# revdotcom/paper_accurate_fast_cheap

Hardware: AMD Instinct MI355X
Metric: audio-sec/sec (1/RTF) GigaSpeech long-form encode (higher is better)
Workload: dtype f32+bf16-slot

## Files before the change

include/pafc_encoder_ops.h:

```cpp
#ifndef PAFC_ENCODER_OPS_H
#define PAFC_ENCODER_OPS_H

#include "pafc_wkv6.h"

#ifdef __cplusplus
extern "C" {
#endif

int pafc_dwconv1d_cl(int dtype, int B, int T_in, int C, int K, int left_pad, int T_out, const void *x,
                     const void *w, const void *bias, void *y, int glu, const int32_t *lens,
                     pafc_stream_t stream);

int pafc_dwconv1d_cl_ex(int dtype, int B, int T_in, int C, int K, int left_pad, int T_out, const void *x, long ldx,
                        const void *w, const void *bias, void *y, int act, const int32_t *lens, pafc_stream_t stream);

int pafc_dwconv1d_cl_ln_silu(int dtype, int B, int T_in, int C, int K, int left_pad, int T_out, const void *x, long ldx,
                             const void *w, const void *bias, const void *gamma, const void *beta, float eps, void *y,
                             const int32_t *lens, pafc_stream_t stream);

size_t pafc_dwconv1d_cl_wgrad_workspace_bytes(int B, int T_out, int C, int K);
int pafc_dwconv1d_cl_wgrad(int dtype, int B, int T_in, int C, int K, int left_pad, int T_out, const void *x, long ldx,
                           const void *dy, float *dw, float *dbias, void *workspace, size_t workspace_bytes,
                           pafc_stream_t stream);

// ... 143 lines not shown
size_t pafc_mamba2_scan_workspace_bytes(int B, int L, int H, int chunk_len);
int pafc_mamba2_scan(int B, int L, int H, const void *xbc, long ldx, const float *dt, const float *log_a, float *y,
                     int chunk_len, void *workspace, size_t workspace_bytes, pafc_stream_t stream);
int pafc_mamba2_scan_dir(int B, int L, int H, const void *xbc, long ldx, const float *dt, const float *log_a, float *y,
                         int reverse, int chunk_len, void *workspace, size_t workspace_bytes, pafc_stream_t stream);

int pafc_mamba2_scan_skip_bf16(int B, int L, int H, const void *xbc, long ldx, const float *dt, const float *log_a,
                               const float *D, void *y_bf16, int reverse, int chunk_len, void *workspace,
                               size_t workspace_bytes, pafc_stream_t stream);
int pafc_mamba2_gate_norm(int dtype, long rows, int d_inner, const void *y, const void *z, long ld_z,
                          const void *norm_weight, float eps, void *out, pafc_stream_t stream);

int pafc_mamba2_scan_state(int B, int L, int H, const void *xbc, long ldx, const float *dt, const float *log_a, const float *D,
                           float *y_f32, void *y_bf16, const float *s_in, float *s_out, int reverse, int chunk_len,
                           void *workspace, size_t workspace_bytes, pafc_stream_t stream);

int pafc_gemm_bf16(long M, int N, int K, int batch, const void *A, long lda, long strideA, const void *W, long ldw,
                   long strideW, const void *bias, long strideBias, const void *residual, long ldr, long strideR,
                   void *out, long ldo, long strideO, float alpha, int act, pafc_stream_t stream);
int pafc_gemm_bf16_glu_half(long M, int N, int K, int batch);
int pafc_conv3x3s2_nhwc_bf16_ph(int B, int T1, int F1, int Ci, int Co, const void *in, const void *w_tap_co_ci, const void *bias,
                                void *out, int relu, int tile_m, pafc_stream_t stream);
int pafc_gemm_bf16_ph(long M, int N, int K, int batch, const void *A, long lda, long strideA, const void *W, long ldw,
                      long strideW, const void *bias, long strideBias, const void *residual, long ldr, long strideR,
                      void *out, long ldo, long strideO, float alpha, int act, int tile_n, int tile_m, pafc_stream_t stream);
int pafc_gemm_ph_ex(long M, int N, int K, int batch, const void *A, long lda, long strideA, int a_split, const void *W, long ldw,
                    long strideW, const void *bias, long strideBias, const void *residual, int res_kind, long ldr, long strideR,
                    void *out, int out_kind, long ldo, long lo_off, long strideO, float alpha, int act, int tile_m,
                    pafc_stream_t stream);
int pafc_gemm_ph_ex2(long M, int N, int K, int batch, const void *A, long lda, long strideA, int a_split, int a_plane_block,
                     const void *W, long ldw, long strideW, const void *bias, long strideBias, const void *residual, int res_kind,
                     long ldr, long strideR, void *out, int out_kind, long ldo, long lo_off, long strideO, float alpha, int act,
                     int tile_m, pafc_stream_t stream);
int pafc_conv3x3s2_nhwc_split_ph(int B, int T1, int F1, int Ci, int Co, const void *in_planes, const void *w3_tap_co_3ci,
                                 const float *bias, void *out_planes, int relu, int tile_m, pafc_stream_t stream);

int pafc_residual_dropout(int backward, int dtype_x, int dtype_y, long n, const void *x, const void *y, void *out, float scale,
                          float p, unsigned long long seed, unsigned long long offset, pafc_stream_t stream);
int pafc_silu_dropout(int backward, int dtype, long n, const void *h, const void *dout, void *out, float p,
                      unsigned long long seed, unsigned long long offset, pafc_stream_t stream);

int pafc_multi_transpose_bf16(const void *table, int n, int total_tiles, pafc_stream_t stream);
int pafc_multi_cast_bf16(const void *table, int n, int total_chunks, pafc_stream_t stream);

#ifdef __cplusplus
}
#endif
#endif
```

paper_accurate_fast_cheap_amd/_lib.py:

```python
import ctypes
import os
from ctypes import c_float, c_int, c_long, c_size_t, c_ulonglong, c_void_p

import torch

_HERE = os.path.dirname(os.path.abspath(__file__))
SO_PATH = os.path.join(_HERE, "libpafc_hip.so")

PAFC_F32, PAFC_BF16 = 0, 1
_ERRORS = {
    -1: "null pointer", -2: "bad dims (B, T, C, H must be positive and C == H * 64)", -3: "head size must be 64",
    -4: "workspace too small", -5: "kernel launch failed", -6: "unsupported dtype", -7: "unsupported",
    -8: "r, k, v, w, y must be 16-byte aligned",
}


class PafcError(RuntimeError):
    pass


_lib = None


def lib():
# ... 58 lines not shown
    "pafc_conv3x3s2_c1_nhwc_f32split": (I, [I, I, I, I, P, P, P, P, P, I, P]),
    "pafc_conv3x3s2_c1_nhwc_f32split_ps": (I, [I, I, I, I, P, P, P, P, P, G, I, P]),
    "pafc_conv3x3s2_nhwc_f32split": (I, [I, I, I, I, I, P, P, P, P, P, P, I, P]),
    "pafc_gemm_tn_workspace_bytes": (Z, [G, I, I]),
    "pafc_gemm_tn_bf16": (I, [G, I, I, P, G, P, G, P, P, I, P, Z, P]),
    "pafc_gemm_tn_batched_workspace_bytes": (Z, [G, I, I, I]),
    "pafc_gemm_tn_bf16_batched": (I, [G, I, I, I, P, G, G, P, G, G, P, P, I, P, Z, P]),
    "pafc_gemm_bf16_f32out": (I, [G, I, I, P, G, I, P, G, P, P, G, P, I, G, G, F, I, P, Z, P]),
    "pafc_gemm_bf16_f32out_pb": (I, [G, I, I, P, G, I, I, P, G, P, P, G, P, I, G, G, F, I, P, Z, P]),
    "pafc_gemm_bf16_f32out_workspace_bytes": (Z, [G, I, I, I]),
    "pafc_ctc_loss_workspace_bytes": (Z, [I, I, I]),
    "pafc_ctc_loss_forward": (I, [I, I, I, I, P, G, P, P, I, P, I, I, P, P, Z, P]),
    "pafc_ctc_loss_backward": (I, [I, I, I, I, P, G, P, P, I, P, I, I, P, P, F, P, G, P, Z, P]),
    "pafc_rnnt_joint_loss_workspace_bytes": (Z, [I, I, I, G, G, P, I]),
    "pafc_rnnt_joint_loss_forward": (I, [I, I, I, I, I, P, G, G, P, G, G, P, P, P, P, P, I, I, G, P, P, Z, P]),
    "pafc_rnnt_joint_loss_backward": (I, [I, I, I, I, I, P, G, G, P, G, G, P, P, P, P, P, I, I, G, P, G, P, F, I, P, P, P, P,
        P, Z, P, Z, P]),
    "pafc_gemm_f32": (I, [G, I, I, I, P, G, G, P, G, G, P, G, P, G, G, P, G, G, F, I, P]),
    "pafc_mamba2_prep": (I, [I, I, I, I, P, P, G, P, P, P, P, P, P, P, P, P]),
    "pafc_mamba2_finish": (I, [I, I, I, I, P, P, P, P, G, P, G, P, P, P, F, I, P, P]),
    "pafc_mamba2_scan_chunk_len": (I, [I, I, I]),
    "pafc_mamba2_scan_workspace_bytes": (Z, [I, I, I, I]),
    "pafc_mamba2_scan": (I, [I, I, I, P, G, P, P, P, I, P, Z, P]),
    "pafc_mamba2_scan_dir": (I, [I, I, I, P, G, P, P, P, I, I, P, Z, P]),
    "pafc_mamba2_scan_skip_bf16": (I, [I, I, I, P, G, P, P, P, P, I, I, P, Z, P]),
    "pafc_mamba2_gate_norm": (I, [I, G, I, P, P, G, P, F, P, P]),
    "pafc_mamba2_scan_state": (I, [I, I, I, P, G, P, P, P, P, P, P, P, I, I, P, Z, P]),
    "pafc_gemm_bf16": (I, [G, I, I, I, P, G, G, P, G, G, P, G, P, G, G, P, G, G, F, I, P]),
    "pafc_gemm_bf16_glu_half": (I, [G, I, I, I]),
    "pafc_conv3x3s2_nhwc_bf16_ph": (I, [I, I, I, I, I, P, P, P, P, I, I, P]),
    "pafc_gemm_bf16_ph": (I, [G, I, I, I, P, G, G, P, G, G, P, G, P, G, G, P, G, G, F, I, I, I, P]),
    "pafc_gemm_ph_ex": (I, [G, I, I, I, P, G, G, I, P, G, G, P, G, P, I, G, G, P, I, G, G, G, F, I, I, P]),
    "pafc_gemm_ph_ex2": (I, [G, I, I, I, P, G, G, I, I, P, G, G, P, G, P, I, G, G, P, I, G, G, G, F, I, I, P]),
    "pafc_conv3x3s2_nhwc_split_ph": (I, [I, I, I, I, I, P, P, P, P, I, I, P]),
    "pafc_residual_dropout": (I, [I, I, I, G, P, P, P, F, F, U, U, P]),
    "pafc_silu_dropout": (I, [I, I, G, P, P, P, F, U, U, P]),
    "pafc_multi_transpose_bf16": (I, [P, I, I, P]),
    "pafc_multi_cast_bf16": (I, [P, I, I, P]),
    "pafc_fbank_num_frames": (G, [G]),
    "pafc_fbank_tables_cols": (I, []),
    "pafc_fbank_f32": (I, [P, G, P, P, P, P, P, I, P, F, F, P, P]),
    "pafc_ctc_greedy": (I, [I, I, I, I, P, P, I, P, P, P, P, P]),
    "pafc_log_softmax_rows": (I, [I, G, I, P, P, P]),
    "pafc_ctc_prefix_beam_workspace_bytes": (Z, [I, I, I]),
    "pafc_ctc_prefix_beam_search": (I, [I, I, I, P, P, P, I, I, P, P, P, P, Z, P]),
    "pafc_ctc_prefix_beam_ex_workspace_bytes": (Z, [I, I, I]),
    "pafc_ctc_prefix_beam_search_ex": (I, [I, I, I, P, P, P, I, I, P, P, P, P, P, P, Z, P]),
    "pafc_ctc_beam_stream_workspace_bytes": (Z, [I, I, I, I]),
    "pafc_ctc_beam_stream_reset": (I, [I, I, I, I, P, P, Z, P]),
    "pafc_ctc_beam_stream_feed": (I, [I, I, I, P, P, P, I, I, I, P, I, P, Z, P]),
    "pafc_ctc_beam_stream_drain": (I, [I, I, I, P, I, P, Z, P, I, P, P, P, P, P, P, I, P, P, P]),
    "pafc_ctc_greedy_stream_workspace_bytes": (Z, [I]),
    "pafc_ctc_greedy_stream_reset": (I, [I, P, P, Z, P]),
    "pafc_ctc_greedy_stream": (I, [I, I, I, I, P, P, I, P, Z, P, P, P, P, P]),
    "pafc_ctc_align_workspace_bytes": (Z, [I, I, I]),
    "pafc_ctc_align": (I, [I, I, I, I, P, G, P, P, I, P, I, P, Z, P, P, P, I, P, P, P]),
    "pafc_rnnt_beam_workspace_bytes": (Z, [I, I, I]),
    "pafc_rnnt_beam_init": (I, [I, I, I, I, P, Z, P, P, P]),
    "pafc_rnnt_beam_step": (I, [I, I, I, I, I, P, P, P, P, P, Z, P, P, P]),
    "pafc_rnnt_beam_finish": (I, [I, I, I, P, Z, P, P, P, P]),
    "pafc_rnnt_beam_stream_workspace_bytes": (Z, [I, I, I]),
    "pafc_rnnt_beam_stream_reset": (I, [I, I, I, I, P, P, Z, P, P, P]),
    "pafc_rnnt_beam_stream_feed": (I, [I, I, I, I, P, P, Z, P]),
    "pafc_rnnt_beam_stream_step": (I, [I, I, I, I, I, I, P, P, P, P, Z, P, P, P]),
    "pafc_rnnt_beam_stream_drain": (I, [I, I, I, P, Z, P, I, P, P, P, P, P, P, P]),
    "pafc_rnnt_beam_select_state": (I, [I, I, I, I, I, P, P, P, P, P, P]),
# ... 70 lines not shown
```

paper_accurate_fast_cheap_amd/csrc/gemm_bf16.hip:

```cpp
#include <stdio.h>
#include <stdlib.h>

#include "pafc_common.h"
#include "../../include/pafc_encoder_ops.h"

namespace pafc {
namespace {

constexpr int GBM = 128, GBN = 128, GBK = 64;
typedef float f32x4g __attribute__((ext_vector_type(4)));
typedef __bf16 bf16x8g __attribute__((ext_vector_type(8)));

struct GemmParams {
    const bf16_t *A, *W, *bias, *res;
    bf16_t *out;
    long M;
    int N, K;
    long lda, ldw, ldo, ldr;
    long sA, sW, sO, sB, sR;
    float alpha;
    int act;
    int mtiles, ntiles;
    int nk1, K1;
    int pb_sh;
// ... 274 lines not shown
        constexpr int LDO = BN + 8;
        bf16_t *O = lds;
#pragma unroll
        for (int j = 0; j < NI; ++j) {
            const int col = wn * (BN / 2) + j * 16 + fr;
            const float bv = bz ? bf16_bits_to_f32(bz[min(n0 + col, p.N - 1)]) : 0.f;
#pragma unroll
            for (int i = 0; i < MI; ++i)
#pragma unroll
                for (int g = 0; g < 4; ++g)
                    O[(wm * (BM / 2) + i * 16 + 4 * kq + g) * LDO + col] =
                        (bf16_t)f32_to_bf16_bits(apply_act(fmaf(acc[i][j][g], p.alpha, bv), p.act));
        }
        __syncthreads();
        constexpr int CPR = BN / 8, RPP = 256 / CPR;
#pragma unroll
        for (int q = 0; q < BM / RPP; ++q) {
            const int row = q * RPP + tid / CPR, c8 = (tid % CPR) * 8;
            const long m = m0 + row;
            if (m < p.M && n0 + c8 < p.N)
                *reinterpret_cast<uint4 *>(Oz + m * p.ldo + n0 + c8) = *reinterpret_cast<const uint4 *>(O + row * LDO + c8);
        }
    }
}

}
}

extern "C" int pafc_gemm_bf16_ph(long M, int N, int K, int batch, const void *A, long lda, long strideA, const void *W, long ldw,
                                 long strideW, const void *bias, long strideBias, const void *residual, long ldr, long strideR,
                                 void *out, long ldo, long strideO, float alpha, int act, int tile_n, int tile_m,
                                 pafc_stream_t stream);

static int ph_tile_m(long M, int N, int K, int batch, int act, bool has_residual) {
    if (N % 8 || K % 128 || N < 256) return 0;
    if (act == 4 && N % 256) return 0;
    if (has_residual && act != 0) return 0;
    const int cus = pafc::device_cus();
    const long nt = (N + 255) / 256;
    static const long min_fill = [] { const char *e = getenv("PAFC_PH_MIN_FILL"); return e ? atol(e) : 0L; }();
    if (min_fill > 0) {
        if (((M + 255) / 256) * nt * batch * 100 < (long)cus * min_fill) return 0;
    } else if (((M + 127) / 128) * ((N + 127) / 128) * batch <= 2L * cus) {
        return 0;
    }
    long best_cost = -1;
    int best = 0;
    for (int tm = 256; tm >= 192; tm -= 64) {
        const long tiles = ((M + tm - 1) / tm) * nt * batch;
        const long cost = ((tiles + cus - 1) / cus) * (tm + 64);
        if (best_cost < 0 || cost < best_cost) { best_cost = cost; best = tm; }
    }
    return best;
}

extern "C" int pafc_gemm_bf16_glu_half(long M, int N, int K, int batch) { return ph_tile_m(M, N, K, batch, 4, false) ? 32 : 64; }

extern "C" int pafc_gemm_bf16(long M, int N, int K, int batch, const void *A, long lda, long strideA, const void *W,
                              long ldw, long strideW, const void *bias, long strideBias, const void *residual, long ldr,
                              long strideR, void *out, long ldo, long strideO, float alpha, int act,
                              pafc_stream_t stream) {
    if (!A || !W || !out) return PAFC_ERR_NULL_POINTER;
    if (M <= 0 || N <= 0 || K <= 0 || batch <= 0 || batch > 65535) return PAFC_ERR_BAD_DIMS;
    if (N % 8 || K % pafc::GBK) return PAFC_ERR_UNSUPPORTED;
    if (act < 0 || act > 4) return PAFC_ERR_UNSUPPORTED;
    if (const int tm = ph_tile_m(M, N, K, batch, act, residual != nullptr)) {
        const int rc = pafc_gemm_bf16_ph(M, N, K, batch, A, lda, strideA, W, ldw, strideW, bias, strideBias, residual, ldr, strideR,
                                         out, ldo, strideO, alpha, act, 256, tm, stream);
        if (rc != PAFC_ERR_UNSUPPORTED) return rc;
        if (act == 4) return PAFC_ERR_UNSUPPORTED;
    }
    const bool glu = act == 4;
    if (glu && (N % pafc::GBN || residual)) return PAFC_ERR_UNSUPPORTED;
    if (lda < K || ldw < K || ldo < (glu ? N / 2 : N) || (residual && ldr < N)) return PAFC_ERR_BAD_DIMS;
    if ((lda | ldw | ldo | strideA | strideW | strideO) % 8 || (residual && ((ldr | strideR) % 8))) return PAFC_ERR_ALIGNMENT;
    if ((((uintptr_t)A | (uintptr_t)W | (uintptr_t)out | (uintptr_t)residual) & 15) != 0) return PAFC_ERR_ALIGNMENT;
    pafc::GemmParams p{};
    p.A = (const pafc::bf16_t *)A; p.W = (const pafc::bf16_t *)W; p.bias = (const pafc::bf16_t *)bias;
    p.res = (const pafc::bf16_t *)residual; p.out = (pafc::bf16_t *)out;
    p.M = M; p.N = N; p.K = K;
    p.lda = lda; p.ldw = ldw; p.ldo = ldo; p.ldr = ldr;
    p.sA = strideA; p.sW = strideW; p.sO = strideO; p.sB = strideBias; p.sR = strideR;
    p.alpha = alpha; p.act = act;
    const long cus = pafc::device_cus();
    auto tiles = [&](int bm, int bn) { return ((M + bm - 1) / bm) * ((N + bn - 1) / bn) * (long)batch; };
    int bm = 128, bn = 128;
// ... 190 lines not shown
```

paper_accurate_fast_cheap_amd/csrc/gemm_ph.hip:

```cpp
#include <climits>
#include <cstdlib>
#include <cstring>
#include <type_traits>

#include "pafc_common.h"
#include "../../include/pafc_encoder_ops.h"

namespace pafc {
namespace {

typedef float f32x4p __attribute__((ext_vector_type(4)));
typedef __bf16 bf16x8p __attribute__((ext_vector_type(8)));
typedef unsigned u32x4p __attribute__((ext_vector_type(4)));

struct PhParams {
    const bf16_t *A, *W;
    const void *bias;
    const void *res;
    void *out;
    long M;
    int N, K;
    long lda, ldw, ldo, ldr;
    long sA, sW, sO, sB, sR;
    float alpha;
// ... 38 lines not shown
template <int ACT>
__device__ __forceinline__ float act_apply(float v) {
    if constexpr (ACT == 1) return v * __builtin_amdgcn_rcpf(1.f + __expf(-v));
    if constexpr (ACT == 2) return 1.f - 2.f * __builtin_amdgcn_rcpf(__expf(2.f * v) + 1.f);
    if constexpr (ACT == 3) return fmaxf(v, 0.f);
    return v;
}

#ifndef PH_ST_AUX
#define PH_ST_AUX 0
#endif
#define PH_WAIT(N) asm volatile("s_waitcnt vmcnt(" #N ")" ::: "memory")
template <int N>
__device__ __forceinline__ void wait_vm() {
    static_assert(N >= 0 && N < 64, "vmcnt is a 6-bit counter");
    asm volatile("s_waitcnt vmcnt(%0)" ::"n"(N) : "memory");
}

constexpr int PBN = 256, PBK = 64;
constexpr unsigned PH_OOB = 0xC0000000u;

template <bool GLU, int ACT, int RES, int OUT, bool CONV = false, int LNF = 0, bool SPL = false>
__global__ __launch_bounds__(512, 2) void gemm_ph_kernel(const PhParams p) {
    constexpr int BN = PBN;
    constexpr int UA = 128 * 128;
    constexpr int UB = (BN / 2) * 128;
    constexpr int STEP = 2 * UA + 2 * UB;
    constexpr int OFF_A0 = 0, OFF_A1 = UA, OFF_B0 = 2 * UA, OFF_B1 = 2 * UA + UB;
    constexpr int TN = 2;
    constexpr int DA = UA / 8192;
    constexpr int DB = UB / 8192;
    constexpr int OSZ = OUT == 1 ? 4 : 2;
    constexpr bool BIASF32 = OUT != 0;
    constexpr int NST = 8 * (GLU ? 1 : 2) * (OUT == 0 ? 1 : 2) + (LNF == 2 ? 8 : 0);
    static_assert(LNF == 0 || (OUT == 0 && !CONV), "LayerNorm folding: bf16 GEMMs");
    static_assert(!SPL || LNF == 0, "shared-fragment split operands: not with a folded LayerNorm");
    static_assert(LNF != 1 || (RES == 0 && (GLU || ACT == 1)), "LNF 1: the w_1 (SiLU) / pointwise_conv1 (GLU) projections");
    static_assert(LNF != 2 || RES == 1, "LNF 2: a residual GEMM");
    static_assert(!(GLU && (ACT != 0 || RES != 0)), "GLU excludes an activation and a residual");
    static_assert(!(RES != 0 && ACT != 0), "the layer never pairs a residual with an activation");
    extern __shared__ __attribute__((aligned(1024))) unsigned char lds[];

    const int tid = threadIdx.x, lane = tid & 63;
    const int wave = __builtin_amdgcn_readfirstlane(tid >> 6);
    const int wr = wave >> 2, wc = wave & 3;
    const long nblk = (long)p.mtiles * p.ntiles;
    const long total = nblk * p.batch;
    const long per = total / 8;
    const int nt = SPL ? p.nsteps : p.K / PBK;

    auto pix_off = [&](long m) -> long {
        const long tf = (long)p.T2 * p.F2;
        const long bb = m / tf, rem = m - bb * tf;
        const long t2 = rem / p.F2, f2 = rem - t2 * p.F2;
        return (((bb * p.T1 + 2 * t2) * p.F1 + 2 * f2) * p.CiA) * 2;
    };

    struct Tile {
        long m0;
        int n0, z, vr;
        __amdgpu_buffer_rsrc_t Ar, Wr;
    };
    auto make_tile = [&](long t, Tile &T) {
        const bool real = t < total;
        long tt = real ? t : 0;
        if (tt < per * 8) tt = (tt % 8) * per + tt / 8;
        T.z = (int)(tt / nblk);
        const long bid = tt % nblk;
        const int mt0 = (int)(bid / p.ntiles), nt0 = (int)(bid % p.ntiles);
        T.m0 = (long)mt0 * p.tm;
        T.n0 = nt0 * BN;
        T.vr = (int)min((long)p.tm, p.M - T.m0);
        if constexpr (CONV) {
            const long a_base = pix_off(T.m0);
            T.Ar = make_rsrc(reinterpret_cast<const unsigned char *>(p.A) + a_base, real ? p.in_bytes - a_base : 0);
            T.Wr = make_rsrc(p.W + (long)T.n0 * p.CiW, real ? ((long)8 * p.N + p.N - T.n0) * p.CiW * 2 : 0);
        } else {
            T.Ar = make_rsrc(p.A + T.z * p.sA + T.m0 * p.lda, real ? (p.M - T.m0) * p.lda * 2 : 0);
            T.Wr = make_rsrc(p.W + T.z * p.sW + (long)T.n0 * p.ldw, real ? ((long)(p.N - 1 - T.n0) * p.ldw + p.K) * 2 : 0);
        }
    };

    unsigned a_off[2][DA], b_off[2][DB];
    auto a_offsets = [&](const Tile &T, int h) {
        int sl = lane;
        asm volatile("" : "+v"(sl));
        const int sub = sl >> 3, pch = sl & 7;
#pragma unroll
        for (int j = 0; j < DA; ++j) {
            const int u = (wave * DA + j) * 8 + sub;
            const int row = (u >> 6) * 128 + h * 64 + (u & 63);
            const int sc = pch ^ sub;
            const unsigned coff = SPL ? (unsigned)(16 * (sc & 3) + (sc >> 2) * p.a_lo) : (unsigned)(16 * sc);
            a_off[h][j] = CONV ? (unsigned)(pix_off(T.m0 + row) - pix_off(T.m0)) + coff
                               : (unsigned)((long)row * p.lda * 2) + coff;
        }
    };
    auto b_offsets = [&]() {
        const int sub = lane >> 3, pch = lane & 7;
#pragma unroll
        for (int h = 0; h < 2; ++h)
#pragma unroll
            for (int j = 0; j < DB; ++j) {
                const int u = (wave * DB + j) * 8 + sub;
                const int r = u & 31;
                const int pc = ((r & 15) >> 2) * 8 + (r >> 4) * 4 + (r & 3);
                const int sc = pch ^ sub;
                const unsigned coff = SPL ? (unsigned)(16 * (sc & 3) + (sc >> 2) * p.w_lo) : (unsigned)(16 * sc);
                b_off[h][j] = (unsigned)((long)((u >> 5) * 64 + h * 32 + pc) * (CONV ? p.CiW : p.ldw) * 2) + coff;
            }
    };
    auto a_soff = [&](int kt) -> unsigned {
        if constexpr (SPL && !CONV) {
            const int blk = kt >> p.pb_shift, c = kt - (blk << p.pb_shift);
            return (unsigned)(blk * 2 * p.pb_bytes + c * 64);
        } else if constexpr (SPL) {
            const int tap = (kt * p.inv_spt) >> 16, kc = kt - tap * p.spt;
            const int dt = (tap * 11) >> 5, df = tap - 3 * dt;
            return (unsigned)(((dt * p.F1 + df) * p.CiA) * 2 + kc * 64);
        } else if constexpr (!CONV) {
            const int seg = (kt >= p.nk1) + (kt >= 2 * p.nk1);
            const int r = kt - seg * p.nk1;
            const int blk = r >> p.pb_shift, c = r - (blk << p.pb_shift);
            return (unsigned)(blk * 2 * p.pb_bytes + (seg == 1 ? p.pb_bytes : 0) + c * 128);
        } else {
            const int tap = (kt * p.inv_spt) >> 16, kc = kt - tap * p.spt;
            const int seg = (kc >= p.nk1) + (kc >= 2 * p.nk1), cc = kc - seg * p.nk1;
            const int dt = (tap * 11) >> 5, df = tap - 3 * dt;
// ... 52 lines not shown
    };

    Tile cur, nxt;
    make_tile(blockIdx.x, cur);
    a_offsets(cur, 0);
    a_offsets(cur, 1);
    b_offsets();
    stage_a(cur, 0, 0, 0); stage_b(cur, 0, 0, 0); stage_b(cur, 1, 0, 0); stage_a(cur, 1, 0, 0);
    stage_a(cur, 0, 1, 1); stage_b(cur, 0, 1, 1);
    __builtin_amdgcn_sched_barrier(0);
    wait_vm<8>();
    __builtin_amdgcn_sched_barrier(0);
    bool first = true;

    for (long t = blockIdx.x; t < total; t += gridDim.x) {
#ifdef PH_STAMPS
    const bool stamp_on = (wave == 0 || wave == 4) && lane == 0 && cur.z == 0;
    unsigned long long *st = p.stamps + ((size_t)t * 2 + (wave >> 2)) * 64;
    PH_STAMP(0);
#endif
    make_tile(CONV ? total : t + gridDim.x, nxt);
    if constexpr (CONV) {
        if (!first) {
            a_offsets(cur, 0);
            a_offsets(cur, 1);
            stage_a(cur, 0, 0, 0); stage_b(cur, 0, 0, 0); stage_b(cur, 1, 0, 0); stage_a(cur, 1, 0, 0);
            stage_a(cur, 0, 1, 1); stage_b(cur, 0, 1, 1);
            __builtin_amdgcn_sched_barrier(0);
            wait_vm<8>();
            __builtin_amdgcn_sched_barrier(0);
        }
    }
    const bool after_stores = !CONV && !first;
    const bool half_on[2] = {wr * 128 < cur.vr, wr * 128 + 64 < cur.vr};
    constexpr int NBL = LNF == 1 ? 4 : 1;
    {
        const long esz = BIASF32 ? 4 : 2;
        const __amdgpu_buffer_rsrc_t Br = make_rsrc(reinterpret_cast<const unsigned char *>(p.bias) + ((long)cur.z * p.sB + cur.n0) * esz,
                                                    p.bias ? (long)(p.N - cur.n0) * esz : 0);
        dma16(Br, lane * 16, 0, lds + 2 * STEP + wave * 1024);
        if constexpr (LNF == 1) {
            const __amdgpu_buffer_rsrc_t Cr = make_rsrc(p.ln_csum + cur.n0, (long)(p.N - cur.n0) * 4);
            dma16(Cr, lane * 16, 0, lds + 2 * STEP + 8 * 1024 + wave * 1024);
        }
    }

    f32x4p acc[2][2][4][TN];
#pragma unroll
    for (int a = 0; a < 2; ++a)
#pragma unroll
        for (int b = 0; b < 2; ++b)
#pragma unroll
            for (int i = 0; i < 4; ++i)
#pragma unroll
                for (int j = 0; j < TN; ++j) acc[a][b][i][j] = f32x4p{0.f, 0.f, 0.f, 0.f};

    auto mma = [&](int mi, int nj, const bf16x8p (&bqf)[TN][2]) {
        __builtin_amdgcn_s_setprio(1);
#ifdef PH_ABL_NOMFMA
        if (false) {
#else
        if (half_on[mi]) {
#endif
            if constexpr (SPL) {
#pragma unroll
                for (int pr = 0; pr < 3; ++pr)
#pragma unroll
                    for (int i = 0; i < 4; ++i)
#pragma unroll
                        for (int j = 0; j < TN; ++j)
                            acc[mi][nj][i][j] = __builtin_amdgcn_mfma_f32_16x16x32_bf16(bqf[j][pr == 2], af[i][pr == 1], acc[mi][nj][i][j], 0, 0, 0);
            } else {
#pragma unroll
                for (int ks = 0; ks < 2; ++ks)
#pragma unroll
                    for (int i = 0; i < 4; ++i)
#pragma unroll
                        for (int j = 0; j < TN; ++j)
                            acc[mi][nj][i][j] = __builtin_amdgcn_mfma_f32_16x16x32_bf16(bqf[j][ks], af[i][ks], acc[mi][nj][i][j], 0, 0, 0);
            }
        }
        __builtin_amdgcn_s_setprio(0);
    };

#ifdef PH_ABL_NOBAR
#define PH_BAR1() do { } while (0)
#else
#define PH_BAR1() __builtin_amdgcn_s_barrier()
#endif
#ifdef PH_ABL_NOEND
#define PH_BAR2() do { } while (0)
#else
#define PH_BAR2() __builtin_amdgcn_s_barrier()
#endif
#define PH_SYNC()                                                                  \
    do {                                                                           \
        if (kt == 0) { if (after_stores) wait_vm<8 + NST + NBL>(); else wait_vm<8 + NBL>(); } \
        else wait_vm<8>();                                                         \
        PH_BAR1();                                                                 \
        __builtin_amdgcn_sched_barrier(0);                                         \
    } while (0)
#define PH_END()                                                                   \
    do {                                                                           \
        __builtin_amdgcn_sched_barrier(0);                                         \
        PH_BAR2();                                                                 \
        __builtin_amdgcn_sched_barrier(0);                                         \
    } while (0)

    auto kstep = [&](auto parc, int kt) {
        constexpr int PAR = decltype(parc)::value;
        const int last = nt - 1 - kt;
        read_b(0, PAR, bf0);
        read_a(0, PAR);
        if (last >= 1) stage_b(cur, 1, PAR ^ 1, kt + 1);
// ... 279 lines not shown
    return hipGetLastError() == hipSuccess ? PAFC_OK : PAFC_ERR_LAUNCH;
}

int g_split_walk = -1;
bool split_shared_fragments() {
    if (g_split_walk < 0) {
        const char *e = getenv("PAFC_SPLIT_WALK");
        g_split_walk = !(e && std::strcmp(e, "hilohi") == 0);
    }
    return g_split_walk != 0;
}

}
}

extern "C" int pafc_gemm_ph_ex(long M, int N, int K, int batch, const void *A, long lda, long strideA, int a_split, const void *W,
                               long ldw, long strideW, const void *bias, long strideBias, const void *residual, int res_kind,
                               long ldr, long strideR, void *out, int out_kind, long ldo, long lo_off, long strideO, float alpha,
                               int act, int tile_m, pafc_stream_t stream) {
    return pafc_gemm_ph_ex2(M, N, K, batch, A, lda, strideA, a_split, 0, W, ldw, strideW, bias, strideBias, residual, res_kind, ldr,
                            strideR, out, out_kind, ldo, lo_off, strideO, alpha, act, tile_m, stream);
}

extern "C" int pafc_gemm_ph_ex2(long M, int N, int K, int batch, const void *A, long lda, long strideA, int a_split,
                                int a_plane_block, const void *W, long ldw, long strideW, const void *bias, long strideBias,
                                const void *residual, int res_kind, long ldr, long strideR, void *out, int out_kind, long ldo,
                                long lo_off, long strideO, float alpha, int act, int tile_m, pafc_stream_t stream) {
    if (!A || !W || !out) return PAFC_ERR_NULL_POINTER;
    if (M <= 0 || N <= 0 || K <= 0 || batch <= 0 || batch > 65535) return PAFC_ERR_BAD_DIMS;
    if (act < 0 || act > 4 || out_kind < 0 || out_kind > 2 || res_kind < 0 || res_kind > 2) return PAFC_ERR_UNSUPPORTED;
    if (!residual) res_kind = 0;
    else if (res_kind == 0) return PAFC_ERR_BAD_DIMS;
    const bool glu = act == 4;
    if (tile_m < 64 || tile_m > 256 || tile_m % 64) return PAFC_ERR_UNSUPPORTED;
    if (N % 8 || K % 128) return PAFC_ERR_UNSUPPORTED;
    if (glu && (N % 256 || residual)) return PAFC_ERR_UNSUPPORTED;
    if (residual && act != 0) return PAFC_ERR_UNSUPPORTED;
    if (res_kind == 1 && out_kind != 0) return PAFC_ERR_UNSUPPORTED;
    if (res_kind == 2 && out_kind != 1) return PAFC_ERR_UNSUPPORTED;
    const int Kw = a_split ? 3 * K : K;
    const int No = glu ? N / 2 : N;
    if (lda < (a_split ? 2 * K : K) || ldw < Kw || (residual && ldr < N)) return PAFC_ERR_BAD_DIMS;
    if (out_kind == 2 ? (lo_off < No || ldo < lo_off + No) : ldo < No) return PAFC_ERR_BAD_DIMS;
    if ((lda | ldw | strideA | strideW) % 8 || (ldo | strideO | lo_off) % 8 || (residual && ((ldr | strideR) % 8))) return PAFC_ERR_ALIGNMENT;
    if ((((uintptr_t)A | (uintptr_t)W | (uintptr_t)out | (uintptr_t)residual | (uintptr_t)bias) & 15) != 0) return PAFC_ERR_ALIGNMENT;
    if ((double)M * lda * 2 >= 2.0e9 || (double)N * ldw * 2 >= 2.0e9) return PAFC_ERR_UNSUPPORTED;
    if ((double)256 * ldo * 4 >= 2.0e9 || (residual && (double)256 * ldr * 4 >= 2.0e9)) return PAFC_ERR_UNSUPPORTED;
    pafc::PhParams p{};
    p.A = (const pafc::bf16_t *)A; p.W = (const pafc::bf16_t *)W; p.bias = bias; p.res = residual; p.out = out;
    p.M = M; p.N = N; p.K = Kw;
    p.lda = lda; p.ldw = ldw; p.ldo = ldo; p.ldr = ldr;
    p.sA = strideA; p.sW = strideW; p.sO = strideO; p.sB = strideBias; p.sR = strideR;
    p.alpha = alpha;
    p.nk1 = a_split ? K / 64 : INT_MAX / 4;
    p.pb_shift = 31;
    p.pb_bytes = (long)K * 2;
    if (a_split && a_plane_block) {
        int sh = 0;
        while ((64 << sh) < a_plane_block) ++sh;
        if ((64 << sh) != a_plane_block || K % a_plane_block) return PAFC_ERR_UNSUPPORTED;
        p.pb_shift = sh;
        p.pb_bytes = (long)a_plane_block * 2;
    }
    p.lo_off = lo_off;
    p.tm = tile_m;
    p.mtiles = (int)((M + tile_m - 1) / tile_m);
    p.ntiles = (N + 255) / 256;
// ... 142 lines not shown
```

paper_accurate_fast_cheap_amd/hip_ops.py:

```python
import contextlib
import ctypes
import math
import os
import threading
import weakref
from typing import List, Optional

import torch

from . import _lib
from ._lib import c_int, c_void_p
from .utils import graph_step


DISPATCH = dict(skinny_max_rows=640, own_gemm_min_rows=1, lds_resident_min_rows=8192, split_gemm_min_rows=1024,
                ln_fold_min_rows=24576, dwconv_ln_silu_max_rows=24575, split_small_max_rows=8192, split_layers_min_rows=256)


def _load_dispatch():
    legacy = dict(skinny_max_rows="PAFC_SKINNY_MAX_ROWS", own_gemm_min_rows="PAFC_OWN_GEMM_MIN_ROWS",
                  lds_resident_min_rows="PAFC_LDS_RESIDENT_MIN_ROWS", split_gemm_min_rows="PAFC_SPLIT_GEMM_MIN_ROWS")
    for name, env in legacy.items():
        if os.environ.get(env):
            DISPATCH[name] = int(os.environ[env])
    for item in filter(None, os.environ.get("PAFC_DISPATCH", "").split(",")):
        name, _, value = item.partition("=")
        if name.strip() not in DISPATCH:
            raise ValueError(f"PAFC_DISPATCH: unknown threshold {name!r} (known: {sorted(DISPATCH)})")
        DISPATCH[name.strip()] = int(value)


_load_dispatch()


# ... 1349 lines not shown
            raise _lib.PafcError("gemm_bf16_ln: 2-d bf16 GPU tensors with unit stride in the last dimension")
    M, K = a.shape
    N = w.shape[0]
    No = N // 2 if act == "glu" else N
    if stats.dtype != torch.float32 or stats.numel() != M * 16 or not stats.is_contiguous():
        raise _lib.PafcError("gemm_bf16_ln: stats is a contiguous float32 (M, 8, 2) buffer")
    if out is None:
        out = torch.empty((M, No), dtype=a.dtype, device=a.device)
    L = _lib.lib()
    from .profiling import op_timer
    with op_timer("gemm_%dx%d" % (K, N), sample=12, flops=2.0 * M * N * K):
        rc = L.pafc_gemm_bf16_ph_ln(M, N, K, _lib.ptr(a), a.stride(0), _lib.ptr(w), w.stride(0), _lib.ptr(bias), _lib.ptr(residual),
                                    residual.stride(0) if residual is not None else 0, _lib.ptr(out), out.stride(0), float(alpha),
                                    _ACTS[act], 1 if csum is not None else 2, _lib.ptr(stats), _lib.ptr(csum),
                                    int(ln_c or (K if csum is not None else N)),
                                    float(eps), _ph_tile_m(M, N, min_tm=128), _lib.stream_of(a))
    _lib.check(rc, "pafc_gemm_bf16_ph_ln")
    return out


def split_planes(x: torch.Tensor, triple: bool = False) -> torch.Tensor:
    _lib.require_gpu(x)
    if x.dtype != torch.float32 or x.stride(-1) != 1:
        raise _lib.PafcError("split_planes: contiguous fp32 input")
    K = x.shape[-1]
    rows = x.numel() // K
    out = torch.empty(x.shape[:-1] + ((3 if triple else 2) * K,), dtype=torch.bfloat16, device=x.device)
    L = _lib.lib()
    _lib.check(L.pafc_split_planes(rows, K, _lib.ptr(x), K, _lib.ptr(out), out.shape[-1], K, int(triple), _lib.stream_of(x)),
               "pafc_split_planes")
    return out


def _ph_tile_m(M: int, N: int, batch: int = 1, min_tm: int = 64) -> int:
    cus = torch.cuda.get_device_properties(torch.cuda.current_device()).multi_processor_count
    nt = (N + 255) // 256
    best = None
    for tm in (256, 192, 128, 64):
        if tm < min_tm:
            continue
        tiles = ((M + tm - 1) // tm) * nt * batch
        cost = ((tiles + cus - 1) // cus) * (tm + 64)
        if best is None or cost < best[0]:
            best = (cost, tm)
    return best[1]


def gemm_ph_ex(a: torch.Tensor, w: torch.Tensor, bias: Optional[torch.Tensor] = None, act: str = "none", alpha: float = 1.0,
               residual: Optional[torch.Tensor] = None, out: Optional[torch.Tensor] = None, a_split: bool = False,
               out_kind: str = "bf16", tile_m: int = 0, a_plane_block: int = 0) -> torch.Tensor:
    _lib.require_gpu(bias)
    for t in (a, w, residual, out):
        if t is not None and (not t.is_cuda or t.stride(-1) != 1):
            raise _lib.PafcError("gemm_ph_ex: GPU tensors with unit stride in the last dimension")
    if a.dtype != torch.bfloat16 or w.dtype != torch.bfloat16 or a.dim() != 2 or w.dim() != 2:
        raise _lib.PafcError("gemm_ph_ex: a and w are 2-d bf16 (planes of fp32 operands with a_split)")
    M = a.shape[0]
    N = w.shape[0]
    K = w.shape[1] // 3 if a_split else w.shape[1]
    if a.shape[1] != (2 * K if a_split else K) or (a_split and w.shape[1] != 3 * K):
        raise _lib.PafcError("gemm_ph_ex: a (M, K) x w (N, K); split: a (M, 2K) x w (N, 3K)")
    No = N // 2 if act == "glu" else N
    kinds = {"bf16": (0, torch.bfloat16, No), "f32": (1, torch.float32, No), "planes": (2, torch.bfloat16, 2 * No)}
    ok, odt, ocols = kinds[out_kind]
    if out is None:
        out = torch.empty((M, ocols), dtype=odt, device=a.device)
    if out.dtype != odt or tuple(out.shape) != (M, ocols):
        raise _lib.PafcError("gemm_ph_ex: out must be (M, N) in the output form's dtype ((M, 2N) bf16 for planes)")
    rk = 0
    if residual is not None:
        rk = 1 if residual.dtype == torch.bfloat16 else 2
        if tuple(residual.shape) != (M, N) or residual.dtype != (torch.bfloat16 if ok == 0 else torch.float32) or ok == 2:
            raise _lib.PafcError("gemm_ph_ex: residual (M, N) in the output dtype (bf16 / fp32), not with planes")
    if bias is not None and (bias.dtype != (torch.bfloat16 if ok == 0 else torch.float32) or bias.numel() != N):
        raise _lib.PafcError("gemm_ph_ex: bias (N) bf16 for a bf16 output, fp32 otherwise")
    L = _lib.lib()
    from .profiling import op_timer
    pb_ok = not a_plane_block or (a_split and a_plane_block >= 64 and a_plane_block & (a_plane_block - 1) == 0 and K % a_plane_block == 0)
    if (M <= _SPLIT_SMALL_MAX_ROWS and M * N <= _SPLIT_SMALL_MAX_OUT and ok != 0 and act in ("none", "silu", "tanh", "relu")
            and pb_ok and not tile_m and K % 64 == 0):
        nws = L.pafc_gemm_bf16_f32out_workspace_bytes(M, N, K, int(a_split))
        ws = torch.empty(nws, dtype=torch.uint8, device=a.device) if nws else None
        with op_timer("gemm%ss_%dx%d" % ("3" if a_split else "", K, N), sample=12, flops=2.0 * M * N * K * (3 if a_split else 1)):
            rc = L.pafc_gemm_bf16_f32out_pb(M, N, K, _lib.ptr(a), a.stride(0), int(a_split), int(a_plane_block), _lib.ptr(w), w.stride(0),
                                            _lib.ptr(bias), _lib.ptr(residual), residual.stride(0) if residual is not None else 0,
                                            _lib.ptr(out), ok, out.stride(0), No if ok == 2 else 0, float(alpha), _ACTS[act], _lib.ptr(ws),
                                            nws, _lib.stream_of(a))
        _lib.check(rc, "pafc_gemm_bf16_f32out")
        return out
    with op_timer("gemm%s_%dx%d" % ("3" if a_split else "", K, N), sample=12, flops=2.0 * M * N * K * (3 if a_split else 1)):
        rc = L.pafc_gemm_ph_ex2(M, N, K, 1, _lib.ptr(a), a.stride(0), 0, int(a_split), int(a_plane_block), _lib.ptr(w), w.stride(0), 0,
                                _lib.ptr(bias), 0,
                               _lib.ptr(residual), rk, residual.stride(0) if residual is not None else 0, 0, _lib.ptr(out), ok,
                               out.stride(0), No if ok == 2 else 0, 0, float(alpha), _ACTS[act], int(tile_m or _ph_tile_m(M, N)),
                               _lib.stream_of(a))
    _lib.check(rc, "pafc_gemm_ph_ex")
    return out


_SPLIT_SMALL_MAX_ROWS = DISPATCH["split_small_max_rows"]
_SPLIT_SMALL_MAX_OUT = 1 << 22


def wkv6_single_chunk(B: int, T: int, C: int, H: int) -> bool:
    return _lib.lib().pafc_wkv6_pick_chunk_len(B, T, C, H, 1) >= T


def _check_prev(prev: Optional[torch.Tensor], x: torch.Tensor):
    if prev is not None and (prev.dtype != x.dtype or prev.numel() != x.shape[0] * x.shape[2] or not prev.is_contiguous()
                             or prev.device != x.device):
        raise _lib.PafcError("tmix: prev must be a contiguous (B, C) tensor of x's dtype on x's device")


def tmix_shift_mix(x: torch.Tensor, maa_x0: torch.Tensor, maa_x1: Optional[torch.Tensor], reverse0: bool = False,
                   prev: Optional[torch.Tensor] = None):
    _lib.require_gpu(x, maa_x0, maa_x1, prev)
    _check_prev(prev, x)
    B, T, C = x.shape
    ndir = 2 if maa_x1 is not None else 1
    out = torch.empty((ndir, B, T, C), dtype=x.dtype, device=x.device)
    rc = _lib.lib().pafc_tmix_shift_mix_prev(_lib.dtype_code(x.dtype), B, T, C, ndir, int(reverse0), _lib.ptr(x),
                                             _lib.ptr(maa_x0), _lib.ptr(maa_x1), _lib.ptr(prev), _lib.ptr(out), _lib.stream_of(x))
    _lib.check(rc, "pafc_tmix_shift_mix")
    return out


def tmix_mix4(x: torch.Tensor, m: torch.Tensor, maa: torch.Tensor, reverse0: bool = False):
# ... 1113 lines not shown
```

Before: 47340.

## Allow 16-row tile_m granularity in ph GEMM with fixed-cost-aware tile picker

Moves the tile_m selection into a shared C function that first picks a multiple of 64 by wave-rounds cost. It then refines in 16-row steps using per-epilogue fixed-overhead estimates, requiring a minimum projected gain. The kernel now accepts tile_m in multiples of 16: rows beyond tm get out-of-bounds load offsets, and the MFMA loop skips dead 16-row groups on the fine path. The goal is less wave quantization and fewer wasted MFMAs on partial tiles, at the cost of extra per-group branching inside the inner MMA loop.

```diff
diff --git a/include/pafc_encoder_ops.h b/include/pafc_encoder_ops.h
--- a/include/pafc_encoder_ops.h
+++ b/include/pafc_encoder_ops.h
@@ -199,6 +199,9 @@
                      const void *W, long ldw, long strideW, const void *bias, long strideBias, const void *residual, int res_kind,
                      long ldr, long strideR, void *out, int out_kind, long ldo, long lo_off, long strideO, float alpha, int act,
                      int tile_m, pafc_stream_t stream);
+enum { PAFC_PH_EPI_BF16 = 0, PAFC_PH_EPI_BF16_RES = 1, PAFC_PH_EPI_F32 = 2, PAFC_PH_EPI_F32_RES = 3, PAFC_PH_EPI_PLANES = 4,
+       PAFC_PH_EPI_GLU = 5 };
+int pafc_gemm_ph_tile_m(long M, int N, int K, int batch, int a_split, int epilogue, int cus, int step, int min_tm);
 int pafc_conv3x3s2_nhwc_split_ph(int B, int T1, int F1, int Ci, int Co, const void *in_planes, const void *w3_tap_co_3ci,
                                  const float *bias, void *out_planes, int relu, int tile_m, pafc_stream_t stream);
 
diff --git a/paper_accurate_fast_cheap_amd/_lib.py b/paper_accurate_fast_cheap_amd/_lib.py
--- a/paper_accurate_fast_cheap_amd/_lib.py
+++ b/paper_accurate_fast_cheap_amd/_lib.py
@@ -114,6 +114,7 @@
     "pafc_gemm_bf16_ph": (I, [G, I, I, I, P, G, G, P, G, G, P, G, P, G, G, P, G, G, F, I, I, I, P]),
     "pafc_gemm_ph_ex": (I, [G, I, I, I, P, G, G, I, P, G, G, P, G, P, I, G, G, P, I, G, G, G, F, I, I, P]),
     "pafc_gemm_ph_ex2": (I, [G, I, I, I, P, G, G, I, I, P, G, G, P, G, P, I, G, G, P, I, G, G, G, F, I, I, P]),
+    "pafc_gemm_ph_tile_m": (I, [G, I, I, I, I, I, I, I, I]),
     "pafc_conv3x3s2_nhwc_split_ph": (I, [I, I, I, I, I, P, P, P, P, I, I, P]),
     "pafc_residual_dropout": (I, [I, I, I, G, P, P, P, F, F, U, U, P]),
     "pafc_silu_dropout": (I, [I, I, G, P, P, P, F, U, U, P]),
diff --git a/paper_accurate_fast_cheap_amd/csrc/gemm_bf16.hip b/paper_accurate_fast_cheap_amd/csrc/gemm_bf16.hip
--- a/paper_accurate_fast_cheap_amd/csrc/gemm_bf16.hip
+++ b/paper_accurate_fast_cheap_amd/csrc/gemm_bf16.hip
@@ -330,6 +330,34 @@
                                  void *out, long ldo, long strideO, float alpha, int act, int tile_n, int tile_m,
                                  pafc_stream_t stream);
 
+static const int PH_FINE_MIN_TM = 160, PH_FINE_MIN_GAIN_PCT = 2;
+static const int PH_FIXED_ROWS[2][6] = {
+    {  280,      0,        0,    446,      0,       0 },
+    {    0,      0,        0,    278,    283,     177 },
+};
+
+extern "C" int pafc_gemm_ph_tile_m(long M, int N, int K, int batch, int a_split, int epilogue, int cus, int step, int min_tm) {
+    if (M <= 0 || N <= 0 || K <= 0 || batch <= 0 || cus <= 0 || epilogue < 0 || epilogue > 5) return 0;
+    if (step != 16 && step != 32 && step != 64) return 0;
+    if (min_tm < 64) min_tm = 64;
+    const long nt = (N + 255) / 256;
+    auto rounds = [&](int tm) { return (((M + tm - 1) / tm) * nt * batch + cus - 1) / cus; };
+    long best_cost = -1;
+    int best = 0;
+    for (int tm = 256; tm >= min_tm; tm -= 64) {
+        const long cost = rounds(tm) * (tm + 64);
+        if (best_cost < 0 || cost < best_cost) { best_cost = cost; best = tm; }
+    }
+    const int fixed = PH_FIXED_ROWS[a_split != 0][epilogue];
+    if (step == 64 || fixed == 0 || best < PH_FINE_MIN_TM) return best;
+    double fine_cost = (double)rounds(best) * (best + fixed) * (100 - PH_FINE_MIN_GAIN_PCT) / 100.0;
+    for (int tm = 256; tm >= (min_tm > PH_FINE_MIN_TM ? min_tm : PH_FINE_MIN_TM); tm -= step) {
+        const double cost = (double)rounds(tm) * (tm + fixed);
+        if (cost < fine_cost) { fine_cost = cost; best = tm; }
+    }
+    return best;
+}
+
 static int ph_tile_m(long M, int N, int K, int batch, int act, bool has_residual) {
     if (N % 8 || K % 128 || N < 256) return 0;
     if (act == 4 && N % 256) return 0;
@@ -342,14 +370,8 @@
     } else if (((M + 127) / 128) * ((N + 127) / 128) * batch <= 2L * cus) {
         return 0;
     }
-    long best_cost = -1;
-    int best = 0;
-    for (int tm = 256; tm >= 192; tm -= 64) {
-        const long tiles = ((M + tm - 1) / tm) * nt * batch;
-        const long cost = ((tiles + cus - 1) / cus) * (tm + 64);
-        if (best_cost < 0 || cost < best_cost) { best_cost = cost; best = tm; }
-    }
-    return best;
+    return pafc_gemm_ph_tile_m(M, N, K, batch, 0, act == 4 ? PAFC_PH_EPI_GLU : has_residual ? PAFC_PH_EPI_BF16_RES : PAFC_PH_EPI_BF16, cus,
+                               16, 192);
 }
 
 extern "C" int pafc_gemm_bf16_glu_half(long M, int N, int K, int batch) { return ph_tile_m(M, N, K, batch, 4, false) ? 32 : 64; }
diff --git a/paper_accurate_fast_cheap_amd/csrc/gemm_ph.hip b/paper_accurate_fast_cheap_amd/csrc/gemm_ph.hip
--- a/paper_accurate_fast_cheap_amd/csrc/gemm_ph.hip
+++ b/paper_accurate_fast_cheap_amd/csrc/gemm_ph.hip
@@ -94,6 +94,7 @@
     constexpr int DB = UB / 8192;
     constexpr int OSZ = OUT == 1 ? 4 : 2;
     constexpr bool BIASF32 = OUT != 0;
+    constexpr bool FINE = !CONV && LNF == 0;
     constexpr int NST = 8 * (GLU ? 1 : 2) * (OUT == 0 ? 1 : 2) + (LNF == 2 ? 8 : 0);
     static_assert(LNF == 0 || (OUT == 0 && !CONV), "LayerNorm folding: bf16 GEMMs");
     static_assert(!SPL || LNF == 0, "shared-fragment split operands: not with a folded LayerNorm");
@@ -156,6 +157,8 @@
             const unsigned coff = SPL ? (unsigned)(16 * (sc & 3) + (sc >> 2) * p.a_lo) : (unsigned)(16 * sc);
             a_off[h][j] = CONV ? (unsigned)(pix_off(T.m0 + row) - pix_off(T.m0)) + coff
                                : (unsigned)((long)row * p.lda * 2) + coff;
+            if constexpr (FINE)
+                if (row >= p.tm) a_off[h][j] = PH_OOB;
         }
     };
     auto b_offsets = [&]() {
@@ -274,7 +277,7 @@
         }
     }
     const bool after_stores = !CONV && !first;
-    const bool half_on[2] = {wr * 128 < cur.vr, wr * 128 + 64 < cur.vr};
+    const int live_g[2] = {min(4, max(0, (cur.vr - wr * 128 + 15) >> 4)), min(4, max(0, (cur.vr - wr * 128 - 64 + 15) >> 4))};
     constexpr int NBL = LNF == 1 ? 4 : 1;
     {
         const long esz = BIASF32 ? 4 : 2;
@@ -299,29 +302,32 @@
 
     auto mma = [&](int mi, int nj, const bf16x8p (&bqf)[TN][2]) {
         __builtin_amdgcn_s_setprio(1);
-#ifdef PH_ABL_NOMFMA
-        if (false) {
-#else
-        if (half_on[mi]) {
-#endif
-            if constexpr (SPL) {
-#pragma unroll
-                for (int pr = 0; pr < 3; ++pr)
-#pragma unroll
-                    for (int i = 0; i < 4; ++i)
-#pragma unroll
-                        for (int j = 0; j < TN; ++j)
-                            acc[mi][nj][i][j] = __builtin_amdgcn_mfma_f32_16x16x32_bf16(bqf[j][pr == 2], af[i][pr == 1], acc[mi][nj][i][j], 0, 0, 0);
-            } else {
-#pragma unroll
-                for (int ks = 0; ks < 2; ++ks)
-#pragma unroll
-                    for (int i = 0; i < 4; ++i)
-#pragma unroll
-                        for (int j = 0; j < TN; ++j)
-                            acc[mi][nj][i][j] = __builtin_amdgcn_mfma_f32_16x16x32_bf16(bqf[j][ks], af[i][ks], acc[mi][nj][i][j], 0, 0, 0);
-            }
-        }
+        auto group = [&](int i) {
+#pragma unroll
+            for (int pr = 0; pr < (SPL ? 3 : 2); ++pr)
+#pragma unroll
+                for (int j = 0; j < TN; ++j) {
+                    const int fb = SPL ? pr == 2 : pr, fa = SPL ? pr == 1 : pr;
+                    acc[mi][nj][i][j] = __builtin_amdgcn_mfma_f32_16x16x32_bf16(bqf[j][fb], af[i][fa], acc[mi][nj][i][j], 0, 0, 0);
+                }
+        };
+#ifndef PH_ABL_NOMFMA
+        if constexpr (FINE) {
+#pragma unroll
+            for (int i = 0; i < 4; ++i)
+                if (i < live_g[mi]) group(i);
+        } else if (live_g[mi] > 0) {
+#pragma unroll
+            for (int pr = 0; pr < (SPL ? 3 : 2); ++pr)
+#pragma unroll
+                for (int i = 0; i < 4; ++i)
+#pragma unroll
+                    for (int j = 0; j < TN; ++j) {
+                        const int fb = SPL ? pr == 2 : pr, fa = SPL ? pr == 1 : pr;
+                        acc[mi][nj][i][j] = __builtin_amdgcn_mfma_f32_16x16x32_bf16(bqf[j][fb], af[i][fa], acc[mi][nj][i][j], 0, 0, 0);
+                    }
+        }
+#endif
         __builtin_amdgcn_s_setprio(0);
     };
 
@@ -667,7 +673,7 @@
     if (!residual) res_kind = 0;
     else if (res_kind == 0) return PAFC_ERR_BAD_DIMS;
     const bool glu = act == 4;
-    if (tile_m < 64 || tile_m > 256 || tile_m % 64) return PAFC_ERR_UNSUPPORTED;
+    if (tile_m < 64 || tile_m > 256 || tile_m % 16) return PAFC_ERR_UNSUPPORTED;
     if (N % 8 || K % 128) return PAFC_ERR_UNSUPPORTED;
     if (glu && (N % 256 || residual)) return PAFC_ERR_UNSUPPORTED;
     if (residual && act != 0) return PAFC_ERR_UNSUPPORTED;
diff --git a/paper_accurate_fast_cheap_amd/hip_ops.py b/paper_accurate_fast_cheap_amd/hip_ops.py
--- a/paper_accurate_fast_cheap_amd/hip_ops.py
+++ b/paper_accurate_fast_cheap_amd/hip_ops.py
@@ -1,5 +1,6 @@
 import contextlib
 import ctypes
+import functools
 import math
 import os
 import threading
@@ -1415,18 +1416,18 @@
     return out
 
 
-def _ph_tile_m(M: int, N: int, batch: int = 1, min_tm: int = 64) -> int:
-    cus = torch.cuda.get_device_properties(torch.cuda.current_device()).multi_processor_count
-    nt = (N + 255) // 256
-    best = None
-    for tm in (256, 192, 128, 64):
-        if tm < min_tm:
-            continue
-        tiles = ((M + tm - 1) // tm) * nt * batch
-        cost = ((tiles + cus - 1) // cus) * (tm + 64)
-        if best is None or cost < best[0]:
-            best = (cost, tm)
-    return best[1]
+PH_EPI = {"bf16": 0, "bf16-res": 1, "f32": 2, "f32-res": 3, "planes": 4, "glu": 5}
+
+
+@functools.lru_cache(maxsize=None)
+def _ph_cus(device: int) -> int:
+    return torch.cuda.get_device_properties(device).multi_processor_count
+
+
+def _ph_tile_m(M: int, N: int, batch: int = 1, min_tm: int = 64, K: int = 512, a_split: bool = False, epilogue: str = "bf16",
+               step: int = 64) -> int:
+    return _lib.lib().pafc_gemm_ph_tile_m(M, N, K, batch, int(a_split), PH_EPI[epilogue], _ph_cus(torch.cuda.current_device()),
+                                          step, min_tm)
 
 
 def gemm_ph_ex(a: torch.Tensor, w: torch.Tensor, bias: Optional[torch.Tensor] = None, act: str = "none", alpha: float = 1.0,
@@ -1471,11 +1472,13 @@
                                             nws, _lib.stream_of(a))
         _lib.check(rc, "pafc_gemm_bf16_f32out")
         return out
+    epi = "glu" if act == "glu" else out_kind + "-res" if residual is not None else out_kind
     with op_timer("gemm%s_%dx%d" % ("3" if a_split else "", K, N), sample=12, flops=2.0 * M * N * K * (3 if a_split else 1)):
         rc = L.pafc_gemm_ph_ex2(M, N, K, 1, _lib.ptr(a), a.stride(0), 0, int(a_split), int(a_plane_block), _lib.ptr(w), w.stride(0), 0,
                                 _lib.ptr(bias), 0,
                                _lib.ptr(residual), rk, residual.stride(0) if residual is not None else 0, 0, _lib.ptr(out), ok,
-                               out.stride(0), No if ok == 2 else 0, 0, float(alpha), _ACTS[act], int(tile_m or _ph_tile_m(M, N)),
+                               out.stride(0), No if ok == 2 else 0, 0, float(alpha), _ACTS[act],
+                               int(tile_m or _ph_tile_m(M, N, K=K, a_split=a_split, epilogue=epi, step=16)),
                                _lib.stream_of(a))
     _lib.check(rc, "pafc_gemm_ph_ex")
     return out
```

Result: no change. 47780, median of 6 (+0.9%).
